# UCSC-VLAA/CLIPA

Measured on AMD Instinct MI355X. Metric: image-text pairs/sec (whole job), full training step, higher is better.
Workload: dtype bf16

## Files before the change

clipa_amd/csrc/attention.hip:

```cpp
#include "common.h"
#include "clipa_hip.h"
#include "attention_common.h"
#include "internal_hooks.h"

namespace {

template <int NKT, int DH, bool CAUSAL>
__global__ __launch_bounds__((64 * attn_waves<NKT, DH>()), HD<DH>::WGS) void attn_fwd_kernel(AttnArgs pin) {
  constexpr int LP = NKT * 32, RB = HD<DH>::RB, KS = HD<DH>::KS, DT = HD<DH>::DT;
  extern __shared__ __attribute__((aligned(16))) char smem[];
  constexpr int HPW = WGHeads<NKT>::HPW, WPH = attn_waves<NKT, DH>() / HPW;
  const int tid = threadIdx.x, lane = tid & 63;
  const int wave_wg = __builtin_amdgcn_readfirstlane(tid >> 6);
  const int slot = wave_wg / WPH, wave = wave_wg % WPH;
  char* sK = smem + slot * (2 * LP * RB);
  char* sV = sK + LP * RB;
  constexpr bool STAGE = fwd_stages<NKT, DH>();
  char* stage = smem + HPW * (2 * LP * RB) + wave_wg * Stg<DH>::BYTES;
  const int l31 = lane & 31, hi = lane >> 5, q16 = (lane >> 4) & 1, i16 = lane & 15;
  const long nheads = (long)pin.B * pin.H;
  const long head_raw = (long)blockIdx.x * HPW + slot;
  const bool live = head_raw < nheads;
  const long head = live ? head_raw : nheads - 1;
  const int b = (int)(head / pin.H), h = (int)(head - (long)b * pin.H);
// ... 67 lines not shown

template <int NKT, int DH, bool CAUSAL>
__global__ __launch_bounds__((64 * attn_waves<NKT, DH>()), HD<DH>::WGS) void attn_bwd_kernel(AttnArgs pin) {
  constexpr int LP = NKT * 32, RB = HD<DH>::RB, KS = HD<DH>::KS, DT = HD<DH>::DT;
  extern __shared__ __attribute__((aligned(16))) char smem[];
  constexpr int HPW = WGHeads<NKT>::HPW, WPH = attn_waves<NKT, DH>() / HPW;
  constexpr bool FENCE = DH == 80 && NKT >= 5;
  const int tid = threadIdx.x, lane = tid & 63;
  const int wave_wg = __builtin_amdgcn_readfirstlane(tid >> 6);
  const int slot = wave_wg / WPH, wave = wave_wg % WPH;
  char* img0 = smem + slot * (2 * LP * RB + 3 * LP * 4);
  char* img1 = img0 + LP * RB;
  float* sM = (float*)(img0 + 2 * LP * RB);
  float* sD = sM + 2 * LP;
  constexpr bool STAGE = bwd_stages<NKT, DH>();
  char* stage = smem + HPW * (2 * LP * RB + 3 * LP * 4) + wave_wg * Stg<DH>::BYTES;
  const int l31 = lane & 31, hi = lane >> 5, q16 = (lane >> 4) & 1, i16 = lane & 15;
  const long nheads = (long)pin.B * pin.H;
  const long head_raw = (long)blockIdx.x * HPW + slot;
  const bool live = head_raw < nheads;
  const long head = live ? head_raw : nheads - 1;
  const int b = (int)(head / pin.H), h = (int)(head - (long)b * pin.H);
  ATTN_LOCATE_SEQUENCE
  const size_t hoff = ((size_t)row0 * p.ld_qkv + (size_t)h * DH) * 2;
  const size_t ooff = ((size_t)row0 * p.ld_o + (size_t)h * DH) * 2;
  const unsigned nrec = (unsigned)((long)(p.L - 1) * p.ld_qkv * 2 + DH * 2);
  const unsigned nrec_o = (unsigned)((long)(p.L - 1) * p.ld_o * 2 + DH * 2);
  const __amdgpu_buffer_rsrc_t rsQ = make_rsrc(p.q + hoff, nrec), rsK = make_rsrc(p.k + hoff, nrec),
                               rsV = make_rsrc(p.v + hoff, nrec), rsDO = make_rsrc(p.d_o + ooff, nrec_o),
                               rsO = make_rsrc(p.o_in + ooff, nrec_o);
  const float c = p.scale * 1.4426950408889634f;
  const float* stats = p.stats + stat0 * 2;

  dma_image<DH>(rsK, img0, LP, p.ld_qkv, wave, lane, WPH);
  dma_image<DH>(rsV, img1, LP, p.ld_qkv, wave, lane, WPH);
  bf16x8 fq[KS], fdo[KS], fo[KS];
  load_frags<KS, DH>(rsQ, p.ld_qkv, 32 * wave + l31, hi, fq);
  load_frags<KS, DH>(rsDO, p.ld_o, 32 * wave + l31, hi, fdo);
  load_frags<KS, DH>(rsO, p.ld_o, 32 * wave + l31, hi, fo);
  asm volatile("s_waitcnt vmcnt(0)" ::: "memory");
  __syncthreads();
  for (int qt = wave; qt < NKT; qt += WPH) {
    const int qg = 32 * qt + l31;
    if (qt != wave) {
      load_frags<KS, DH>(rsQ, p.ld_qkv, qg, hi, fq);
      load_frags<KS, DH>(rsDO, p.ld_o, qg, hi, fdo);
      load_frags<KS, DH>(rsO, p.ld_o, qg, hi, fo);
    }
    float mp = 1e30f;
    if (qg < p.L) {
      const float2 st = *(const float2*)(stats + qg * 2);
      mp = st.x - __builtin_amdgcn_logf(st.y);
    }
    float Dq = 0.f;
#pragma unroll
    for (int ks = 0; ks < KS; ++ks) {
      float a[8], o8[8];
      unpack8(__builtin_bit_cast(u32x4, fdo[ks]), a);
      unpack8(__builtin_bit_cast(u32x4, fo[ks]), o8);
#pragma unroll
      for (int i = 0; i < 8; ++i) Dq += a[i] * o8[i];
    }
    Dq += __shfl_xor(Dq, 32, 64);
    if (hi == 0) { sM[qg] = mp; sD[qg] = Dq; }
    const int lim2 = (CAUSAL ? min(p.L, qg + 1) : p.L) - 4 * hi;
    f32x16 dq[DT];
#pragma unroll
    for (int dt = 0; dt < DT; ++dt)
#pragma unroll
      for (int r = 0; r < 16; ++r) dq[dt][r] = 0.f;
#pragma unroll
    for (int kt = 0; kt < NKT; ++kt) {
      if (CAUSAL && kt > qt) continue;
      f32x16 s, dp;
#pragma unroll
      for (int r = 0; r < 16; ++r) { s[r] = 0.f; dp[r] = 0.f; }
#pragma unroll
      for (int ks = 0; ks < KS; ++ks) {
        s = __builtin_amdgcn_mfma_f32_32x32x16_bf16(frag_direct<DH>(img0, 32 * kt, l31, hi, ks), fq[ks], s, 0, 0, 0);
        dp = __builtin_amdgcn_mfma_f32_32x32x16_bf16(frag_direct<DH>(img1, 32 * kt, l31, hi, ks), fdo[ks], dp, 0, 0, 0);
      }
      if constexpr (FENCE) __builtin_amdgcn_sched_barrier(0);
      const bool full = CAUSAL ? ((32 * kt + 32 <= p.L) && kt < qt) : (kt < NKT - 1);
      float ds[16];
#pragma unroll
      for (int r = 0; r < 16; ++r) {
        float pe = __builtin_amdgcn_exp2f(fmaf(s[r], c, -mp));
        if (!full) pe = (32 * kt + 8 * (r >> 2) + (r & 3) < lim2) ? pe : 0.f;
        ds[r] = pe * (dp[r] - Dq);
      }
      if constexpr (FENCE) __builtin_amdgcn_sched_barrier(0);
#pragma unroll
      for (int s2 = 0; s2 < 2; ++s2) {
        const bf16x8 dsf = pack_frag(ds + 8 * s2);
#pragma unroll
        for (int dt = 0; dt < DT; ++dt)
          dq[dt] = __builtin_amdgcn_mfma_f32_32x32x16_bf16(frag_trans<DH>(img0, 32 * kt + 16 * s2, 32 * dt, hi, q16, i16), dsf, dq[dt], 0, 0, 0);
      }
    }
    if constexpr (STAGE) {
      if (live) store_tile<DH>(stage, p.dq, p.ld_dqkv, row0 + 32 * qt, p.L - 32 * qt, h * DH, lane, dq, p.scale);
    } else if (qg < p.L && live) {
#pragma unroll
      for (int dt = 0; dt < DT; ++dt)
        store_frag_T(p.dq, p.ld_dqkv, row0 + qg, h * DH + 32 * dt, hi, dq[dt], p.scale, DH - 32 * dt);
    }
  }
  bf16x8 fk[KS], fv[KS];
#pragma unroll
  for (int ks = 0; ks < KS; ++ks) {
    fk[ks] = frag_direct<DH>(img0, 32 * min(wave, NKT - 1), l31, hi, ks);
    fv[ks] = frag_direct<DH>(img1, 32 * min(wave, NKT - 1), l31, hi, ks);
  }
  asm volatile("s_waitcnt lgkmcnt(0)" ::: "memory");
  __syncthreads();

  dma_image<DH>(rsQ, img0, LP, p.ld_qkv, wave, lane, WPH);
  dma_image<DH>(rsDO, img1, LP, p.ld_o, wave, lane, WPH);
  asm volatile("s_waitcnt vmcnt(0)" ::: "memory");
  __syncthreads();
  for (int kt = wave; kt < NKT; kt += WPH) {
    const int kg = 32 * kt + l31;
    const int kgc = l31 - 4 * hi;
    if (kt != wave) {
      load_frags<KS, DH>(rsK, p.ld_qkv, kg, hi, fk);
      load_frags<KS, DH>(rsV, p.ld_qkv, kg, hi, fv);
    }
    f32x16 dk[DT], dv[DT];
#pragma unroll
    for (int dt = 0; dt < DT; ++dt)
#pragma unroll
      for (int r = 0; r < 16; ++r) { dk[dt][r] = 0.f; dv[dt][r] = 0.f; }
    for (int qt = (CAUSAL ? kt : 0); qt < NKT; ++qt) {
      f32x16 s, dp;
#pragma unroll
      for (int r = 0; r < 16; ++r) { s[r] = 0.f; dp[r] = 0.f; }
#pragma unroll
      for (int ks = 0; ks < KS; ++ks) {
        s = __builtin_amdgcn_mfma_f32_32x32x16_bf16(frag_direct<DH>(img0, 32 * qt, l31, hi, ks), fk[ks], s, 0, 0, 0);
        dp = __builtin_amdgcn_mfma_f32_32x32x16_bf16(frag_direct<DH>(img1, 32 * qt, l31, hi, ks), fv[ks], dp, 0, 0, 0);
      }
      if constexpr (FENCE) __builtin_amdgcn_sched_barrier(0);
      float pr[16], ds[16];
#pragma unroll
      for (int rq = 0; rq < 4; ++rq) {
        const int q0 = 32 * qt + 8 * rq + 4 * hi;
        const float4 m4 = *(const float4*)(sM + q0);
        const float4 d4 = *(const float4*)(sD + q0);
        const float mm[4] = {m4.x, m4.y, m4.z, m4.w};
        const float dd[4] = {d4.x, d4.y, d4.z, d4.w};
#pragma unroll
        for (int e = 0; e < 4; ++e) {
          const int r = 4 * rq + e;
          float pe = __builtin_amdgcn_exp2f(fmaf(s[r], c, -mm[e]));
          if (CAUSAL && qt == kt) pe = (kgc <= 8 * rq + e) ? pe : 0.f;
          pr[r] = pe;
          ds[r] = pe * (dp[r] - dd[e]);
        }
      }
      if constexpr (FENCE) __builtin_amdgcn_sched_barrier(0);
#pragma unroll
      for (int s2 = 0; s2 < 2; ++s2) {
        const bf16x8 pf = pack_frag(pr + 8 * s2);
        const bf16x8 dsf = pack_frag(ds + 8 * s2);
#pragma unroll
        for (int dt = 0; dt < DT; ++dt) {
          dv[dt] = __builtin_amdgcn_mfma_f32_32x32x16_bf16(frag_trans<DH>(img1, 32 * qt + 16 * s2, 32 * dt, hi, q16, i16), pf, dv[dt], 0, 0, 0);
          dk[dt] = __builtin_amdgcn_mfma_f32_32x32x16_bf16(frag_trans<DH>(img0, 32 * qt + 16 * s2, 32 * dt, hi, q16, i16), dsf, dk[dt], 0, 0, 0);
        }
      }
    }
    if constexpr (STAGE) {
      if (live) {
        store_tile<DH>(stage, p.dk, p.ld_dqkv, row0 + 32 * kt, p.L - 32 * kt, h * DH, lane, dk, p.scale);
        store_tile<DH>(stage, p.dv, p.ld_dqkv, row0 + 32 * kt, p.L - 32 * kt, h * DH, lane, dv, 1.0f);
      }
    } else if (kg < p.L && live) {
#pragma unroll
      for (int dt = 0; dt < DT; ++dt) {
        store_frag_T(p.dk, p.ld_dqkv, row0 + kg, h * DH + 32 * dt, hi, dk[dt], p.scale, DH - 32 * dt);
        store_frag_T(p.dv, p.ld_dqkv, row0 + kg, h * DH + 32 * dt, hi, dv[dt], 1.0f, DH - 32 * dt);
      }
    }
  }
}

constexpr int LONG_CT = 8;
constexpr int LONG_LMAX = 1024;

template <int DH>
__device__ __forceinline__ __amdgpu_buffer_rsrc_t chunk_rsrc(const char* base, long ld, int row0, int L) {
  const long rows = (long)L - row0;
  const long bytes = rows > 0 ? (rows - 1) * ld * 2 + DH * 2 : 0;
  return make_rsrc(base + (size_t)row0 * ld * 2, (unsigned)bytes);
}

template <int DH, bool CAUSAL>
__global__ __launch_bounds__(256, HD<DH>::WGS) void attn_fwd_long_kernel(AttnArgs p) {
  constexpr int CT = LONG_CT, RB = HD<DH>::RB, KS = HD<DH>::KS, DT = HD<DH>::DT;
  extern __shared__ __attribute__((aligned(16))) char smem[];
  const int tid = threadIdx.x, lane = tid & 63;
  const int wave = __builtin_amdgcn_readfirstlane(tid >> 6);
  char* sK = smem;
// ... 320 lines not shown
  if (L <= 0 || L > LONG_LMAX) { clipa_set_error("attention: L=%ld outside (0, %d]", (long)L, LONG_LMAX); return CLIPA_ERR_ARG; }
  if (ld_qkv % 8 != 0 || ld_o % 8 != 0) { clipa_set_error("attention: row strides must be multiples of 8 elements"); return CLIPA_ERR_ARG; }
  if (B * H <= 0 || B * H > 0x7fffffffL) { clipa_set_error("attention: bad B*H"); return CLIPA_ERR_ARG; }
  return 0;
}

}

#define ATTN_DISPATCH_DH(fn, DH, a, st)                                     \
  switch (((a).L + 31) / 32) {                                               \
    case 1: return fn<1, DH>(a, st); case 2: return fn<2, DH>(a, st);        \
    case 3: return fn<3, DH>(a, st); case 4: return fn<4, DH>(a, st);        \
    case 5: return fn<5, DH>(a, st); case 6: return fn<6, DH>(a, st);        \
    case 7: return fn<7, DH>(a, st); case 8: return fn<8, DH>(a, st);        \
    default: return fn<9, DH>(a, st);                                        \
  }
#ifdef CLIPA_ATTN_WIDE
template <int NKT, int DH> int wide_fwd(const AttnArgs& a, hipStream_t st) { return launch_fwd_c<NKT, DH, false>(a, st); }
template <int NKT, int DH> int wide_bwd(const AttnArgs& a, hipStream_t st) { return launch_bwd_c<NKT, DH, false>(a, st); }
template <int DH>
int wide_dh(const AttnArgs& a, int bwd, hipStream_t st) {
  if (a.L > 288) return bwd ? launch_long<DH, false, true>(a, st) : launch_long<DH, false, false>(a, st);
  if (bwd) { ATTN_DISPATCH_DH(wide_bwd, DH, a, st) }
  ATTN_DISPATCH_DH(wide_fwd, DH, a, st)
}
extern "C" int clipa_attn_wide_launch(const void* args, int64_t dh, int bwd, void* stream) {
  const AttnArgs& a = *(const AttnArgs*)args;
  if (dh == 88) return wide_dh<88>(a, bwd, (hipStream_t)stream);
  if (dh == 104) return wide_dh<104>(a, bwd, (hipStream_t)stream);
  return wide_dh<112>(a, bwd, (hipStream_t)stream);
}
#else
extern "C" int clipa_attn_wide_launch(const void* args, int64_t dh, int bwd, void* stream);
#ifdef CLIPA_ATTN_PERSISTENT_EXPERIMENT
extern "C" int clipa_attn_bwd1_try(const void* args, int64_t dh, void* stream, int* rc);
extern "C" int clipa_attn_fwd1_try(const void* args, int64_t dh, void* stream, int* rc);
#endif

#define ATTN_DISPATCH(fn, dh, a, st)                 \
  if ((dh) == 80) { ATTN_DISPATCH_DH(fn, 80, a, st) } \
  ATTN_DISPATCH_DH(fn, 64, a, st)

extern "C" int clipa_attention_fwd(const void* q, const void* k, const void* v, void* out, float* stats,
                                   int64_t B, int64_t H, int64_t L, int64_t dh, int64_t ld_qkv, int64_t ld_o,
                                   float scale, int causal, void* stream) {
  if (B * H == 0) return CLIPA_OK;
  if (int rc = check_args(B, H, L, dh, ld_qkv, ld_o, causal)) return rc;
  AttnArgs a = {};
  a.q = (const char*)q; a.k = (const char*)k; a.v = (const char*)v; a.ld_qkv = ld_qkv;
  a.o = (char*)out; a.ld_o = ld_o; a.B = (int)B; a.H = (int)H; a.L = (int)L; a.scale = scale; a.causal = causal;
  a.stats = stats;
  if (wide_head(dh)) return clipa_attn_wide_launch(&a, dh, 0, stream);
  if (L > 288) return dispatch_long<false>(a, dh, (hipStream_t)stream);
#ifdef CLIPA_ATTN_PERSISTENT_EXPERIMENT
  int rc1 = 0;
  if ((clipa_internal_debug_flags() & 524288) && clipa_attn_fwd1_try(&a, dh, stream, &rc1)) return rc1;
#endif
  ATTN_DISPATCH(launch_fwd, dh, a, (hipStream_t)stream)
}

extern "C" int clipa_attention_bwd(const void* q, const void* k, const void* v, const void* out,
                                   const void* d_out, const float* stats, void* dq, void* dk, void* dv, int64_t B, int64_t H,
                                   int64_t L, int64_t dh, int64_t ld_qkv, int64_t ld_o, int64_t ld_dqkv,
                                   float scale, int causal, void* stream) {
  if (B * H == 0) return CLIPA_OK;
  if (int rc = check_args(B, H, L, dh, ld_qkv, ld_o, causal)) return rc;
  if (ld_dqkv % 8 != 0) { clipa_set_error("attention_bwd: ld_dqkv must be a multiple of 8"); return CLIPA_ERR_ARG; }
  if (!stats) { clipa_set_error("attention_bwd: needs the forward's softmax statistics"); return CLIPA_ERR_ARG; }
  AttnArgs a = {};
  a.q = (const char*)q; a.k = (const char*)k; a.v = (const char*)v; a.ld_qkv = ld_qkv;
  a.o_in = (const char*)out; a.d_o = (const char*)d_out; a.ld_o = ld_o;
  a.dq = (char*)dq; a.dk = (char*)dk; a.dv = (char*)dv; a.ld_dqkv = ld_dqkv;
  a.B = (int)B; a.H = (int)H; a.L = (int)L; a.scale = scale; a.causal = causal;
  a.stats = const_cast<float*>(stats);
  if (wide_head(dh)) return clipa_attn_wide_launch(&a, dh, 1, stream);
  if (L > 288) return dispatch_long<true>(a, dh, (hipStream_t)stream);
#ifdef CLIPA_ATTN_PERSISTENT_EXPERIMENT
  int rc1 = 0;
  if ((clipa_internal_debug_flags() & 262144) && clipa_attn_bwd1_try(&a, dh, stream, &rc1)) return rc1;
#endif
  ATTN_DISPATCH(launch_bwd, dh, a, (hipStream_t)stream)
}
namespace {
int varlen_args(const int* seq_start, const int* seq_len, int64_t nseq, int64_t tiles, int64_t dh) {
  if (!seq_start || !seq_len) { clipa_set_error("attention (varlen): seq_start / seq_len missing"); return CLIPA_ERR_ARG; }
  if (tiles < 1 || tiles > 9) { clipa_set_error("attention (varlen): tiles=%ld outside [1, 9] (sequences of up to 288 tokens)", (long)tiles); return CLIPA_ERR_ARG; }
  if (dh != 64 && dh != 80) { clipa_set_error("attention (varlen): head dim %ld unsupported (64 and 80)", (long)dh); return CLIPA_ERR_ARG; }
  (void)nseq;
  return 0;
}
}

extern "C" int clipa_attention_fwd_varlen(const void* q, const void* k, const void* v, void* out, float* stats,
                                          const int32_t* seq_start, const int32_t* seq_len, const int32_t* seq_ids, int64_t nseq,
                                          int64_t tiles, int64_t H, int64_t dh, int64_t ld_qkv, int64_t ld_o, float scale,
                                          int causal, void* stream) {
  if (nseq * H == 0) return CLIPA_OK;
  if (int rc = check_args(nseq, H, 32 * tiles, dh, ld_qkv, ld_o, causal)) return rc;
  if (int rc = varlen_args(seq_start, seq_len, nseq, tiles, dh)) return rc;
  AttnArgs a = {};
  a.q = (const char*)q; a.k = (const char*)k; a.v = (const char*)v; a.ld_qkv = ld_qkv;
  a.o = (char*)out; a.ld_o = ld_o; a.B = (int)nseq; a.H = (int)H; a.L = (int)(32 * tiles); a.scale = scale; a.causal = causal;
  a.stats = stats;
  a.seq_start = seq_start; a.seq_len = seq_len; a.seq_ids = seq_ids;
  ATTN_DISPATCH(launch_fwd, dh, a, (hipStream_t)stream)
}

extern "C" int clipa_attention_bwd_varlen(const void* q, const void* k, const void* v, const void* out, const void* d_out,
                                          const float* stats, void* dq, void* dk, void* dv, const int32_t* seq_start,
                                          const int32_t* seq_len, const int32_t* seq_ids, int64_t nseq, int64_t tiles, int64_t H,
                                          int64_t dh, int64_t ld_qkv, int64_t ld_o, int64_t ld_dqkv, float scale, int causal,
                                          void* stream) {
  if (nseq * H == 0) return CLIPA_OK;
// ... 15 lines not shown
```

clipa_amd/csrc/attention_common.h:

```cpp
#pragma once
#include "common.h"

namespace {

struct AttnArgs {
  const char* q; const char* k; const char* v; long ld_qkv;
  char* o; const char* o_in; const char* d_o; long ld_o;
  char* dq; char* dk; char* dv; long ld_dqkv;
  float* stats;
  int B, H, L;
  float scale;
  int causal;
  const int* seq_start; const int* seq_len; const int* seq_ids;
  int abl;
};

template <int DH>
struct HD {
  static constexpr int RB = DH == 64 ? 128 : 256;
  static constexpr int NCH = RB / 16;
  static constexpr int KS = (DH + 15) / 16;
  static constexpr int DT = (DH + 31) / 32;
  static constexpr int WGS = DH == 64 ? 2 : 1;
};
template <int NKT>
struct WGHeads {
  static constexpr int HPW = NKT == 1 ? 4 : (NKT == 2 ? 2 : 1);
  static constexpr int WPH = 4 / HPW;
};
template <int NKT, int DH>
__host__ __device__ constexpr int attn_waves() { return (DH == 80 && NKT >= 5) ? 8 : 4; }

template <int DH>
__device__ __forceinline__ int swz_u(int row) {
  if (DH == 64) return (((row >> 1) & 1) << 2) | ((row >> 2) & 1) | (((row >> 3) & 1) << 1);
  return ((row & 3) << 2) | ((row >> 2) & 3);
}

template <int DH>
__device__ __forceinline__ void dma_image(const __amdgpu_buffer_rsrc_t rs, char* img, int LP, long ld,
                                          int wave, int lane, int nwaves = 4) {
  constexpr int NCH = HD<DH>::NCH, RPP = 1024 / HD<DH>::RB;
  for (int pc = wave; pc < LP / RPP; pc += nwaves) {
    const int row = pc * RPP + lane / NCH;
    const int chunk = (lane & (NCH - 1)) ^ swz_u<DH>(row);
    const unsigned oob = (chunk * 8 >= DH) ? 0x80000000u : 0u;
    __builtin_amdgcn_raw_ptr_buffer_load_lds(rs, LDS_PTR(img + pc * 1024), 16,
                                             (unsigned)(row * ld * 2 + chunk * 16) | oob, 0, 0, 0);
  }
}

template <int DH>
__device__ __forceinline__ bf16x8 frag_direct(const char* img, int rowbase, int l31, int hi, int ks) {
  return *(const bf16x8*)(img + (rowbase + l31) * HD<DH>::RB + (((2 * ks + hi) ^ swz_u<DH>(l31)) << 4));
}

template <int DH>
__device__ __forceinline__ bf16x8 frag_trans(const char* img, int rowbase16, int colbase, int hi, int q16, int i16) {
  constexpr int RB = HD<DH>::RB;
  const int col = colbase + 16 * q16 + 4 * (i16 & 3);
  const int r0 = rowbase16 + 4 * hi + (i16 >> 2);
  const int r1 = r0 + 8;
  const bf16x4 a = __builtin_amdgcn_ds_read_tr16_b64_v4i16(
      (__attribute__((address_space(3))) bf16x4*)(img + r0 * RB + (((col >> 3) ^ swz_u<DH>(r0)) << 4) + (col & 7) * 2));
  const bf16x4 b = __builtin_amdgcn_ds_read_tr16_b64_v4i16(
      (__attribute__((address_space(3))) bf16x4*)(img + r1 * RB + (((col >> 3) ^ swz_u<DH>(r1)) << 4) + (col & 7) * 2));
  bf16x8 f;
  f[0] = a[0]; f[1] = a[1]; f[2] = a[2]; f[3] = a[3];
  f[4] = b[0]; f[5] = b[1]; f[6] = b[2]; f[7] = b[3];
  return f;
}

__device__ __forceinline__ bf16x8 pack_frag(const float* v) {
  u32x4 w;
#pragma unroll
  for (int i = 0; i < 4; ++i) w[i] = pack2bf(v[2 * i], v[2 * i + 1]);
  return __builtin_bit_cast(bf16x8, w);
}

__device__ __forceinline__ void store_frag_T(char* base, long ld, long row, int col0, int hi, const f32x16& a, float mul,
                                             int ncols = 32) {
#pragma unroll
  for (int qd = 0; qd < 4; ++qd) {
    if (8 * qd >= ncols) continue;
// ... 136 lines not shown
```

clipa_amd/csrc/misc.hip:

```cpp
#include "common.h"
#include "stream.h"
#include "clipa_hip.h"

namespace {

template <int DT>
__global__ void patchify_kernel(const void* __restrict__ img, unsigned short* __restrict__ out,
                                int B, int S, int P, int g, int Kp, int nhwc, int normalize,
                                float m0, float m1, float m2, float is0, float is1, float is2) {
  const long total = (long)B * g * g * (Kp / 8);
  const int K = 3 * P * P;
  const bool fast8 = nhwc && (3 * P) % 8 == 0 && (3 * S) % 8 == 0 && ((size_t)img & 7) == 0;
  for (long idx = (long)blockIdx.x * blockDim.x + threadIdx.x; idx < total; idx += (long)gridDim.x * blockDim.x) {
    const int kc = (int)(idx % (Kp / 8));
    const long patch = idx / (Kp / 8);
    const int px = (int)(patch % g);
    const int py = (int)((patch / g) % g);
    const long b = patch / ((long)g * g);
    float f[8];
    if (DT == 0 && fast8) {
      const int k0 = kc * 8;
      if (k0 < K) {
        const int ph = k0 / (3 * P), off = k0 - ph * 3 * P;
        const size_t src = (((size_t)b * S + (py * P + ph)) * S + px * P) * 3 + off;
// ... 103 lines not shown
template <bool TBF16>
__global__ void embed_tokens_kernel(const long* __restrict__ ids, const void* __restrict__ table,
                                    const float* __restrict__ pos, unsigned short* __restrict__ out,
                                    long B, int T, int D, int vocab, int* __restrict__ oob) {
  const int dc = D / 8;
  const long total = B * T * dc;
  for (long idx = (long)blockIdx.x * blockDim.x + threadIdx.x; idx < total; idx += (long)gridDim.x * blockDim.x) {
    const int c = (int)(idx % dc);
    const long row = idx / dc;
    const int t = (int)(row % T);
    long id = ids[row];
    if (id < 0 || id >= vocab) {
      if (c == 0 && oob) atomicAdd(oob, 1);
      id = 0;
    }
    float v[8], pe[8];
    if (TBF16) {
      unpack8(*(const u32x4*)((const unsigned short*)table + (size_t)id * D + c * 8), v);
    } else {
      *(float4*)v = *(const float4*)((const float*)table + (size_t)id * D + c * 8);
      *(float4*)(v + 4) = *(const float4*)((const float*)table + (size_t)id * D + c * 8 + 4);
#pragma unroll
      for (int i = 0; i < 8; ++i) v[i] = bf2f(f2bf(v[i]));
    }
    *(float4*)pe = *(const float4*)(pos + (size_t)t * D + c * 8);
    *(float4*)(pe + 4) = *(const float4*)(pos + (size_t)t * D + c * 8 + 4);
#pragma unroll
    for (int i = 0; i < 8; ++i) v[i] += bf2f(f2bf(pe[i]));
    *(u32x4*)(out + (size_t)row * D + c * 8) = pack8(v);
  }
}

constexpr double EMB_FIX = 17592186044416.0;
__global__ void embed_tokens_bwd_kernel(const long* __restrict__ ids, const unsigned short* __restrict__ dx,
                                        unsigned long long* __restrict__ acc, unsigned char* __restrict__ bad_row, long B, int T,
                                        int D, int vocab, int* __restrict__ oob) {
  const int dc = D / 8;
  const long total = B * T * dc;
  for (long idx = (long)blockIdx.x * blockDim.x + threadIdx.x; idx < total; idx += (long)gridDim.x * blockDim.x) {
    const int c = (int)(idx % dc);
    const long row = idx / dc;
    const long id = ids[row];
    if (id < 0 || id >= vocab) {
      if (c == 0 && oob) atomicAdd(oob, 1);
      continue;
    }
    const u32x4 raw = *(const u32x4*)(dx + (size_t)row * D + c * 8);
    if (((raw[0] | raw[1] | raw[2] | raw[3]) & 0x7fff7fffu) == 0) continue;
    float v[8];
    unpack8(raw, v);
#pragma unroll
    for (int i = 0; i < 8; ++i) {
      if (v[i] == 0.f) continue;
      if (!(fabsf(v[i]) <= 3.0e38f)) { bad_row[id] = 1; continue; }
      const float vs = fminf(fmaxf(v[i], -131072.0f), 131072.0f);
      atomicAdd(acc + (size_t)id * D + c * 8 + i, (unsigned long long)__double2ll_rn((double)vs * EMB_FIX));
    }
  }
}
__global__ void embed_fix_to_f32_kernel(const long long* __restrict__ acc, const unsigned char* __restrict__ bad_row,
                                        float* __restrict__ out, long n, int D) {
  for (long i = (long)blockIdx.x * blockDim.x + threadIdx.x; i < n; i += (long)gridDim.x * blockDim.x)
    out[i] = bad_row[i / D] ? __int_as_float(0x7fc00000) : (float)((double)acc[i] * (1.0 / EMB_FIX));
}

__global__ void argmax_tokens_kernel(const long* __restrict__ ids, int* __restrict__ out, long B, int T) {
  const long b = (long)blockIdx.x * blockDim.x + threadIdx.x;
  if (b >= B) return;
  long best = ids[b * T];
  int bi = 0;
  for (int t = 1; t < T; ++t) {
    const long v = ids[b * T + t];
    if (v > best) { best = v; bi = t; }
  }
  out[b] = bi;
}

__global__ void pool_fwd_kernel(const unsigned short* __restrict__ x, const int* __restrict__ idx,
                                float* __restrict__ out, long B, int L, int D, int mode) {
  const int dc = D / 8;
  const long total = B * dc;
  for (long i = (long)blockIdx.x * blockDim.x + threadIdx.x; i < total; i += (long)gridDim.x * blockDim.x) {
    const int c = (int)(i % dc);
    const long b = i / dc;
    float acc[8] = {0, 0, 0, 0, 0, 0, 0, 0};
    int l0, l1;
    if (mode == CLIPA_POOL_FIRST) { l0 = 0; l1 = 1; }
    else if (mode == CLIPA_POOL_LAST) { l0 = L - 1; l1 = L; }
    else if (mode == CLIPA_POOL_INDEX) { l0 = idx[b]; l1 = l0 + 1; }
    else if (mode == CLIPA_POOL_MEAN_ALL) { l0 = 0; l1 = L; }
    else { l0 = 1; l1 = L; }
    for (int l = l0; l < l1; ++l) {
      float v[8];
      unpack8(*(const u32x4*)(x + ((size_t)b * L + l) * D + c * 8), v);
#pragma unroll
      for (int k = 0; k < 8; ++k) acc[k] += v[k];
// ... 228 lines not shown
extern "C" int clipa_assemble_tokens_bwd(const void* dtokens, void* dpatch, float* dcls, float* dpos,
                                         int64_t B, int64_t L, int64_t D, void* workspace, int64_t workspace_bytes,
                                         void* stream) {
  if (D % 8 != 0) { clipa_set_error("assemble_tokens_bwd: D%%8 != 0"); return CLIPA_ERR_ARG; }
  if (B <= 0) return CLIPA_OK;
  if (!workspace || workspace_bytes < clipa_assemble_tokens_bwd_workspace(B, L, D)) { clipa_set_error("assemble_tokens_bwd: workspace too small"); return CLIPA_ERR_ARG; }
  hipStream_t st = (hipStream_t)stream;
  int nchunk, bchunk;
  assemble_bwd_chunks(B, L, D, &nchunk, &bchunk);
  const long threads = L * (D / 8);
  hipLaunchKernelGGL(assemble_tokens_bwd_kernel, dim3((unsigned)((threads + 255) / 256), (unsigned)nchunk), dim3(256), 0, st,
                     (const unsigned short*)dtokens, (unsigned short*)dpatch, (float*)workspace, (long)B, (int)L, (int)D, bchunk);
  if (int rc = clipa_check_launch("assemble_tokens_bwd")) return rc;
  if (!dcls && !dpos) return CLIPA_OK;
  const long n = dpos ? L * D : D;
  hipLaunchKernelGGL(assemble_tokens_bwd_reduce_kernel, dim3((unsigned)((n + 255) / 256)), dim3(256), 0, st, (const float*)workspace,
                     dcls, dpos, (int)L, (int)D, nchunk);
  return clipa_check_launch("assemble_tokens_bwd_reduce");
}

extern "C" int clipa_embed_tokens(const int64_t* ids, const void* table, int table_bf16, const float* pos,
                                  void* out, int64_t B, int64_t T, int64_t D, int64_t vocab, int32_t* oob_count,
                                  void* stream) {
  if (D % 8 != 0) { clipa_set_error("embed_tokens: D%%8 != 0"); return CLIPA_ERR_ARG; }
  if (B <= 0) return CLIPA_OK;
  const unsigned grid = grid_for(B * T * (D / 8));
  if (table_bf16) hipLaunchKernelGGL(embed_tokens_kernel<true>, dim3(grid), dim3(256), 0, (hipStream_t)stream, (const long*)ids, table, pos, (unsigned short*)out, (long)B, (int)T, (int)D, (int)vocab, oob_count);
  else hipLaunchKernelGGL(embed_tokens_kernel<false>, dim3(grid), dim3(256), 0, (hipStream_t)stream, (const long*)ids, table, pos, (unsigned short*)out, (long)B, (int)T, (int)D, (int)vocab, oob_count);
  return clipa_check_launch("embed_tokens");
}

extern "C" int64_t clipa_embed_tokens_bwd_workspace(int64_t B, int64_t T, int64_t D, int64_t vocab, int need_table,
                                                   int need_pos) {
  int64_t w = need_table ? vocab * D * (int64_t)sizeof(long long) + (vocab + 7) / 8 * 8 : 0;
  const int64_t pw = need_pos ? clipa_assemble_tokens_bwd_workspace(B, T, D) : 0;
  return w > pw ? w : pw;
}

extern "C" int clipa_embed_tokens_bwd(const int64_t* ids, const void* dx, float* dtable, float* dpos,
                                      int64_t B, int64_t T, int64_t D, int64_t vocab, int32_t* oob_count, void* workspace,
                                      int64_t workspace_bytes, void* stream) {
  if (D % 8 != 0) { clipa_set_error("embed_tokens_bwd: D%%8 != 0"); return CLIPA_ERR_ARG; }
  if (B <= 0) return CLIPA_OK;
  if (!workspace || workspace_bytes < clipa_embed_tokens_bwd_workspace(B, T, D, vocab, dtable != nullptr, dpos != nullptr)) {
    clipa_set_error("embed_tokens_bwd: workspace too small");
    return CLIPA_ERR_ARG;
  }
  hipStream_t st = (hipStream_t)stream;
  if (dtable) {
    unsigned char* bad_row = (unsigned char*)workspace + vocab * D * sizeof(long long);
    (void)hipMemsetAsync(workspace, 0, vocab * D * sizeof(long long) + (vocab + 7) / 8 * 8, st);
    hipLaunchKernelGGL(embed_tokens_bwd_kernel, dim3(grid_for(B * T * (D / 8))), dim3(256), 0, st, (const long*)ids, (const unsigned short*)dx, (unsigned long long*)workspace, bad_row, (long)B, (int)T, (int)D, (int)vocab, oob_count);
    if (int rc = clipa_check_launch("embed_tokens_bwd")) return rc;
    hipLaunchKernelGGL(embed_fix_to_f32_kernel, dim3(grid_for(vocab * D)), dim3(256), 0, st, (const long long*)workspace, bad_row, dtable, (long)(vocab * D), (int)D);
    if (int rc = clipa_check_launch("embed_tokens_bwd_convert")) return rc;
  }
  if (dpos) return clipa_assemble_tokens_bwd(dx, nullptr, nullptr, dpos, B, T, D, workspace, workspace_bytes, stream);
  return CLIPA_OK;
}

extern "C" int clipa_argmax_tokens(const int64_t* ids, int32_t* out, int64_t B, int64_t T, void* stream) {
  if (B <= 0) return CLIPA_OK;
  hipLaunchKernelGGL(argmax_tokens_kernel, dim3((unsigned)((B + 255) / 256)), dim3(256), 0, (hipStream_t)stream, (const long*)ids, out, (long)B, (int)T);
  return clipa_check_launch("argmax_tokens");
}

extern "C" int clipa_pool_fwd(const void* x, const int32_t* idx, float* out, int64_t B, int64_t L, int64_t D,
                              int mode, void* stream) {
  if (D % 8 != 0 || (mode == CLIPA_POOL_INDEX && !idx)) { clipa_set_error("pool_fwd: bad args"); return CLIPA_ERR_ARG; }
  if (B <= 0) return CLIPA_OK;
  hipLaunchKernelGGL(pool_fwd_kernel, dim3(grid_for(B * (D / 8))), dim3(256), 0, (hipStream_t)stream, (const unsigned short*)x, idx, out, (long)B, (int)L, (int)D, mode);
  return clipa_check_launch("pool_fwd");
}
extern "C" int clipa_pool_bwd(const float* dout, const int32_t* idx, void* dx, int64_t B, int64_t L, int64_t D,
                              int mode, void* stream) {
  if (D % 8 != 0 || (mode == CLIPA_POOL_INDEX && !idx)) { clipa_set_error("pool_bwd: bad args"); return CLIPA_ERR_ARG; }
  if (B <= 0) return CLIPA_OK;
  hipLaunchKernelGGL(pool_bwd_kernel, dim3(grid_for(B * L * (D / 8))), dim3(256), 0, (hipStream_t)stream, dout, idx, (unsigned short*)dx, (long)B, (int)L, (int)D, mode);
  return clipa_check_launch("pool_bwd");
}

namespace {
__global__ void gather_rows_kernel(const unsigned short* __restrict__ x, const int64_t* __restrict__ rows,
                                   unsigned short* __restrict__ out, long n_out, long n_src, int D) {
  const int dc = D / 8;
  const long total = n_out * dc;
  for (long idx = (long)blockIdx.x * blockDim.x + threadIdx.x; idx < total; idx += (long)gridDim.x * blockDim.x) {
    const long r = idx / dc;
// ... 252 lines not shown
```

Before: 2468.

## Prefetch next tile fragments and use direct-to-LDS DMA in attention backward

Measured after the change: 2473, median of 6. No clear change (+0.2%).

```diff
diff --git a/clipa_amd/csrc/attention.hip b/clipa_amd/csrc/attention.hip
--- a/clipa_amd/csrc/attention.hip
+++ b/clipa_amd/csrc/attention.hip
@@ -123,8 +123,9 @@
   const float c = p.scale * 1.4426950408889634f;
   const float* stats = p.stats + stat0 * 2;
 
-  dma_image<DH>(rsK, img0, LP, p.ld_qkv, wave, lane, WPH);
-  dma_image<DH>(rsV, img1, LP, p.ld_qkv, wave, lane, WPH);
+  constexpr bool HIDDEN = attn_bwd_hidden_dma<NKT, DH, CAUSAL>();
+  head_image<DH, LP, WPH, HIDDEN>(p.k + hoff, nrec, img0, p.ld_qkv, wave, lane);
+  head_image<DH, LP, WPH, HIDDEN>(p.v + hoff, nrec, img1, p.ld_qkv, wave, lane);
   bf16x8 fq[KS], fdo[KS], fo[KS];
   load_frags<KS, DH>(rsQ, p.ld_qkv, 32 * wave + l31, hi, fq);
   load_frags<KS, DH>(rsDO, p.ld_o, 32 * wave + l31, hi, fdo);
@@ -133,7 +134,7 @@
   __syncthreads();
   for (int qt = wave; qt < NKT; qt += WPH) {
     const int qg = 32 * qt + l31;
-    if (qt != wave) {
+    if (!HIDDEN && qt != wave) {
       load_frags<KS, DH>(rsQ, p.ld_qkv, qg, hi, fq);
       load_frags<KS, DH>(rsDO, p.ld_o, qg, hi, fdo);
       load_frags<KS, DH>(rsO, p.ld_o, qg, hi, fo);
@@ -188,6 +189,11 @@
         for (int dt = 0; dt < DT; ++dt)
           dq[dt] = __builtin_amdgcn_mfma_f32_32x32x16_bf16(frag_trans<DH>(img0, 32 * kt + 16 * s2, 32 * dt, hi, q16, i16), dsf, dq[dt], 0, 0, 0);
       }
+    }
+    if (HIDDEN && qt + WPH < NKT) {
+      load_frags<KS, DH>(rsQ, p.ld_qkv, qg + 32 * WPH, hi, fq);
+      load_frags<KS, DH>(rsDO, p.ld_o, qg + 32 * WPH, hi, fdo);
+      load_frags<KS, DH>(rsO, p.ld_o, qg + 32 * WPH, hi, fo);
     }
     if constexpr (STAGE) {
       if (live) store_tile<DH>(stage, p.dq, p.ld_dqkv, row0 + 32 * qt, p.L - 32 * qt, h * DH, lane, dq, p.scale);
@@ -206,14 +212,14 @@
   asm volatile("s_waitcnt lgkmcnt(0)" ::: "memory");
   __syncthreads();
 
-  dma_image<DH>(rsQ, img0, LP, p.ld_qkv, wave, lane, WPH);
-  dma_image<DH>(rsDO, img1, LP, p.ld_o, wave, lane, WPH);
+  head_image<DH, LP, WPH, HIDDEN>(p.q + hoff, nrec, img0, p.ld_qkv, wave, lane);
+  head_image<DH, LP, WPH, HIDDEN>(p.d_o + ooff, nrec_o, img1, p.ld_o, wave, lane);
   asm volatile("s_waitcnt vmcnt(0)" ::: "memory");
   __syncthreads();
   for (int kt = wave; kt < NKT; kt += WPH) {
     const int kg = 32 * kt + l31;
     const int kgc = l31 - 4 * hi;
-    if (kt != wave) {
+    if (!HIDDEN && kt != wave) {
       load_frags<KS, DH>(rsK, p.ld_qkv, kg, hi, fk);
       load_frags<KS, DH>(rsV, p.ld_qkv, kg, hi, fv);
     }
@@ -260,6 +266,10 @@
           dk[dt] = __builtin_amdgcn_mfma_f32_32x32x16_bf16(frag_trans<DH>(img0, 32 * qt + 16 * s2, 32 * dt, hi, q16, i16), dsf, dk[dt], 0, 0, 0);
         }
       }
+    }
+    if (HIDDEN && kt + WPH < NKT) {
+      load_frags<KS, DH>(rsK, p.ld_qkv, kg + 32 * WPH, hi, fk);
+      load_frags<KS, DH>(rsV, p.ld_qkv, kg + 32 * WPH, hi, fv);
     }
     if constexpr (STAGE) {
       if (live) {
@@ -646,10 +656,6 @@
 }
 #else
 extern "C" int clipa_attn_wide_launch(const void* args, int64_t dh, int bwd, void* stream);
-#ifdef CLIPA_ATTN_PERSISTENT_EXPERIMENT
-extern "C" int clipa_attn_bwd1_try(const void* args, int64_t dh, void* stream, int* rc);
-extern "C" int clipa_attn_fwd1_try(const void* args, int64_t dh, void* stream, int* rc);
-#endif
 
 #define ATTN_DISPATCH(fn, dh, a, st)                 \
   if ((dh) == 80) { ATTN_DISPATCH_DH(fn, 80, a, st) } \
@@ -666,10 +672,6 @@
   a.stats = stats;
   if (wide_head(dh)) return clipa_attn_wide_launch(&a, dh, 0, stream);
   if (L > 288) return dispatch_long<false>(a, dh, (hipStream_t)stream);
-#ifdef CLIPA_ATTN_PERSISTENT_EXPERIMENT
-  int rc1 = 0;
-  if ((clipa_internal_debug_flags() & 524288) && clipa_attn_fwd1_try(&a, dh, stream, &rc1)) return rc1;
-#endif
   ATTN_DISPATCH(launch_fwd, dh, a, (hipStream_t)stream)
 }
 
@@ -689,10 +691,6 @@
   a.stats = const_cast<float*>(stats);
   if (wide_head(dh)) return clipa_attn_wide_launch(&a, dh, 1, stream);
   if (L > 288) return dispatch_long<true>(a, dh, (hipStream_t)stream);
-#ifdef CLIPA_ATTN_PERSISTENT_EXPERIMENT
-  int rc1 = 0;
-  if ((clipa_internal_debug_flags() & 262144) && clipa_attn_bwd1_try(&a, dh, stream, &rc1)) return rc1;
-#endif
   ATTN_DISPATCH(launch_bwd, dh, a, (hipStream_t)stream)
 }
 namespace {
diff --git a/clipa_amd/csrc/attention_common.h b/clipa_amd/csrc/attention_common.h
--- a/clipa_amd/csrc/attention_common.h
+++ b/clipa_amd/csrc/attention_common.h
@@ -1,5 +1,6 @@
 #pragma once
 #include "common.h"
+#include "gemm_common.h"
 
 namespace {
 
@@ -12,7 +13,6 @@
   float scale;
   int causal;
   const int* seq_start; const int* seq_len; const int* seq_ids;
-  int abl;
 };
 
 template <int DH>
@@ -50,6 +50,34 @@
   }
 }
 
+template <int NKT, int DH, bool CAUSAL>
+__host__ __device__ constexpr bool attn_bwd_hidden_dma() { return DH == 64 && NKT >= 3 && !(NKT == 8 && !CAUSAL); }
+
+template <int DH, int LP, int NWAVES>
+__device__ __forceinline__ void dma_image_hidden(const u32x4 srd, char* img, long ld, int wave, int lane) {
+  constexpr int NCH = HD<DH>::NCH, RPP = 1024 / HD<DH>::RB, PIECES = LP / RPP;
+  static_assert(PIECES % NWAVES == 0, "every wave issues the same number of pieces");
+#pragma unroll
+  for (int j = 0; j < PIECES / NWAVES; ++j) {
+    const int pc = wave + j * NWAVES;
+    const int row = pc * RPP + lane / NCH;
+    const int chunk = (lane & (NCH - 1)) ^ swz_u<DH>(row);
+    const unsigned oob = (chunk * 8 >= DH) ? 0x80000000u : 0u;
+    clipa_gemm::dma16(srd, (unsigned)(size_t)LDS_PTR(img + pc * 1024), (unsigned)(row * ld * 2 + chunk * 16) | oob, 0u);
+  }
+}
+template <int DH, int LP, int NWAVES, bool HIDDEN>
+__device__ __forceinline__ void head_image(const char* base, unsigned nrec, char* img, long ld, int wave, int lane) {
+  if constexpr (HIDDEN) {
+    u32x4 srd = clipa_gemm::make_srd(base, nrec);
+#pragma unroll
+    for (int i = 0; i < 4; ++i) srd[i] = __builtin_amdgcn_readfirstlane(srd[i]);
+    dma_image_hidden<DH, LP, NWAVES>(srd, img, ld, wave, lane);
+  } else {
+    dma_image<DH>(make_rsrc(base, nrec), img, LP, ld, wave, lane, NWAVES);
+  }
+}
+
 template <int DH>
 __device__ __forceinline__ bf16x8 frag_direct(const char* img, int rowbase, int l31, int hi, int ks) {
   return *(const bf16x8*)(img + (rowbase + l31) * HD<DH>::RB + (((2 * ks + hi) ^ swz_u<DH>(l31)) << 4));
```

## Replace atomic fixed-point embedding backward with sort-by-token segmented reduction

Applied to the files above, without the earlier changes.

New measurement: 2476 before, 2482 after, median of 6. About the same (+0.2%).

```diff
diff --git a/clipa_amd/csrc/misc.hip b/clipa_amd/csrc/misc.hip
--- a/clipa_amd/csrc/misc.hip
+++ b/clipa_amd/csrc/misc.hip
@@ -159,36 +159,223 @@
 }
 
 constexpr double EMB_FIX = 17592186044416.0;
-__global__ void embed_tokens_bwd_kernel(const long* __restrict__ ids, const unsigned short* __restrict__ dx,
-                                        unsigned long long* __restrict__ acc, unsigned char* __restrict__ bad_row, long B, int T,
-                                        int D, int vocab, int* __restrict__ oob) {
+constexpr int EMB_SEG = 32;
+
+struct EmbBwdWs {
+  int* count;
+  unsigned char* bad;
+  int* rowoff;
+  int* itemoff;
+  int* slotoff;
+  int* item_id;
+  int* rank;
+  int* sorted;
+  long long* partial;
+  int64_t zero_bytes, bytes;
+};
+inline EmbBwdWs emb_bwd_carve(void* ws, int64_t nrows, int64_t D, int64_t vocab) {
+  EmbBwdWs w;
+  int64_t off = 0;
+  auto take = [&](int64_t bytes) { void* p = (void*)((uintptr_t)ws + (uintptr_t)off); off += (bytes + 15) / 16 * 16; return p; };
+  w.count = (int*)take(vocab * 4);
+  w.bad = (unsigned char*)take(vocab);
+  w.zero_bytes = off;
+  w.rowoff = (int*)take((vocab + 1) * 4);
+  w.itemoff = (int*)take((vocab + 1) * 4);
+  w.slotoff = (int*)take((vocab + 1) * 4);
+  w.item_id = (int*)take((vocab + nrows / EMB_SEG) * 4);
+  w.rank = (int*)take(nrows * 4);
+  w.sorted = (int*)take(nrows * 4);
+  w.partial = (long long*)take((2 * nrows / EMB_SEG + 1) * D * (int64_t)sizeof(long long));
+  w.bytes = off;
+  return w;
+}
+
+__global__ void embed_bwd_count_kernel(const long* __restrict__ ids, const unsigned short* __restrict__ dx,
+                                       int* __restrict__ count, int* __restrict__ rank, long nrows, int D, int vocab,
+                                       int* __restrict__ oob) {
+  const int lane = threadIdx.x & 63;
+  const long row = (long)blockIdx.x * blockDim.x + threadIdx.x;
+  const long wbase = row - lane;
   const int dc = D / 8;
-  const long total = B * T * dc;
+  const int nr = (int)(nrows - wbase < 64 ? nrows - wbase : 64);
+  bool live = false;
+#pragma unroll 4
+  for (int k = 0; k < nr; ++k) {
+    unsigned any = 0;
+    for (int c = lane; c < dc; c += 64) {
+      const u32x4 raw = *(const u32x4*)(dx + (size_t)(wbase + k) * D + c * 8);
+      any |= (raw[0] | raw[1] | raw[2] | raw[3]) & 0x7fff7fffu;
+    }
+    const bool nz = __ballot(any != 0) != 0ull;
+    if (lane == k) live = nz;
+  }
+  int id = -1;
+  if (row < nrows) {
+    const long id64 = ids[row];
+    if (id64 < 0 || id64 >= vocab) { if (oob) atomicAdd(oob, 1); }
+    else if (live) id = (int)id64;
+  }
+  int leader = lane, within = 0, gsize = 1;
+  bool todo = id >= 0;
+  for (unsigned long long pending = __ballot(todo); pending; pending = __ballot(todo)) {
+    const int first = __ffsll((long long)pending) - 1;
+    const bool mine = todo && id == __shfl(id, first);
+    const unsigned long long grp = __ballot(mine);
+    if (mine) {
+      leader = first;
+      within = __popcll(grp & ((1ull << lane) - 1ull));
+      gsize = __popcll(grp);
+      todo = false;
+    }
+  }
+  int base = 0;
+  if (id >= 0 && lane == leader) base = atomicAdd(count + id, gsize);
+  base = __shfl(base, leader);
+  if (row < nrows) rank[row] = id >= 0 ? base + within : -1;
+}
+
+__device__ __forceinline__ void emb_block_scan3(int (&v)[3], int (*s)[1024]) {
+  const int t = threadIdx.x;
+#pragma unroll
+  for (int k = 0; k < 3; ++k) s[k][t] = v[k];
+  __syncthreads();
+  for (int d = 1; d < 1024; d <<= 1) {
+    int u[3];
+#pragma unroll
+    for (int k = 0; k < 3; ++k) u[k] = t >= d ? s[k][t - d] : 0;
+    __syncthreads();
+#pragma unroll
+    for (int k = 0; k < 3; ++k) s[k][t] += u[k];
+    __syncthreads();
+  }
+#pragma unroll
+  for (int k = 0; k < 3; ++k) v[k] = s[k][t];
+}
+__device__ __forceinline__ void emb_id_sizes(int n, int (&v)[3]) {
+  const int items = n > EMB_SEG ? (n + EMB_SEG - 1) / EMB_SEG : 1;
+  v[0] = n; v[1] = items; v[2] = items > 1 ? items : 0;
+}
+
+__global__ __launch_bounds__(1024) void embed_bwd_scan_kernel(const int* __restrict__ count, int* __restrict__ rowoff,
+                                                              int* __restrict__ itemoff, int* __restrict__ slotoff,
+                                                              int* __restrict__ item_id, int vocab) {
+  __shared__ int s[3][1024];
+  const int t = threadIdx.x, first = blockIdx.x * 1024, id = first + t;
+  int front[3] = {0, 0, 0};
+  for (int i = t; i < first; i += 1024) {
+    int v[3];
+    emb_id_sizes(count[i], v);
+#pragma unroll
+    for (int k = 0; k < 3; ++k) front[k] += v[k];
+  }
+  emb_block_scan3(front, s);
+  int base[3];
+#pragma unroll
+  for (int k = 0; k < 3; ++k) base[k] = s[k][1023];
+  __syncthreads();
+  int own[3] = {0, 0, 0}, incl[3];
+  if (id < vocab) emb_id_sizes(count[id], own);
+#pragma unroll
+  for (int k = 0; k < 3; ++k) incl[k] = own[k];
+  emb_block_scan3(incl, s);
+  if (id >= vocab) return;
+  const int r = base[0] + incl[0] - own[0], it = base[1] + incl[1] - own[1], sl = base[2] + incl[2] - own[2];
+  rowoff[id] = r;
+  itemoff[id] = it;
+  slotoff[id] = sl;
+  for (int j = 0; j < own[1]; ++j) item_id[it + j] = id;
+  if (id == vocab - 1) { rowoff[vocab] = r + own[0]; itemoff[vocab] = it + own[1]; slotoff[vocab] = sl + own[2]; }
+}
+
+__global__ void embed_bwd_place_kernel(const long* __restrict__ ids, const int* __restrict__ rank,
+                                       const int* __restrict__ rowoff, int* __restrict__ sorted, long nrows) {
+  const long row = (long)blockIdx.x * blockDim.x + threadIdx.x;
+  if (row >= nrows) return;
+  const int r = rank[row];
+  if (r >= 0) sorted[rowoff[ids[row]] + r] = (int)row;
+}
+
+__device__ __forceinline__ void emb_fix_add(const u32x4 raw, long long (&acc)[8], bool& nonfinite) {
+  if (((raw[0] | raw[1] | raw[2] | raw[3]) & 0x7fff7fffu) == 0) return;
+  float v[8];
+  unpack8(raw, v);
+#pragma unroll
+  for (int i = 0; i < 8; ++i) {
+    if (v[i] == 0.f) continue;
+    if (!(fabsf(v[i]) <= 3.0e38f)) { nonfinite = true; continue; }
+    const float vs = fminf(fmaxf(v[i], -131072.0f), 131072.0f);
+    acc[i] = (long long)((unsigned long long)acc[i] + (unsigned long long)__double2ll_rn((double)vs * EMB_FIX));
+  }
+}
+__device__ __forceinline__ void emb_fix_store(const long long (&acc)[8], float* __restrict__ out) {
+  float f[8];
+#pragma unroll
+  for (int i = 0; i < 8; ++i) f[i] = (float)((double)acc[i] * (1.0 / EMB_FIX));
+  *(float4*)out = make_float4(f[0], f[1], f[2], f[3]);
+  *(float4*)(out + 4) = make_float4(f[4], f[5], f[6], f[7]);
+}
+
+__global__ void embed_bwd_sum_kernel(const unsigned short* __restrict__ dx, const int* __restrict__ rowoff,
+                                     const int* __restrict__ itemoff, const int* __restrict__ slotoff,
+                                     const int* __restrict__ item_id, const int* __restrict__ sorted,
+                                     unsigned char* __restrict__ bad, long long* __restrict__ partial,
+                                     float* __restrict__ dtable, int D, int vocab) {
+  const int item = blockIdx.x;
+  if (item >= itemoff[vocab]) return;
+  const int id = item_id[item];
+  const int j = item - itemoff[id], nitems = itemoff[id + 1] - itemoff[id];
+  const int r0 = rowoff[id] + j * EMB_SEG;
+  const int r1 = r0 + EMB_SEG < rowoff[id + 1] ? r0 + EMB_SEG : rowoff[id + 1];
+  const int dc = D / 8;
+  for (int c = threadIdx.x; c < dc; c += blockDim.x) {
+    long long acc[8] = {0, 0, 0, 0, 0, 0, 0, 0};
+    bool nonfinite = false;
+    for (int r = r0; r < r1; r += 4) {
+      u32x4 raw[4];
+#pragma unroll
+      for (int u = 0; u < 4; ++u) {
+        raw[u] = u32x4{0u, 0u, 0u, 0u};
+        if (r + u < r1) raw[u] = *(const u32x4*)(dx + (size_t)sorted[r + u] * D + c * 8);
+      }
+#pragma unroll
+      for (int u = 0; u < 4; ++u) emb_fix_add(raw[u], acc, nonfinite);
+    }
+    if (nonfinite) bad[id] = 1;
+    if (nitems == 1) {
+      emb_fix_store(acc, dtable + (size_t)id * D + c * 8);
+    } else {
+      long long* p = partial + (size_t)(slotoff[id] + j) * D + c * 8;
+#pragma unroll
+      for (int i = 0; i < 8; ++i) p[i] = acc[i];
+    }
+  }
+}
+
+__global__ void embed_bwd_merge_kernel(const int* __restrict__ itemoff, const int* __restrict__ slotoff,
+                                       const unsigned char* __restrict__ bad, const long long* __restrict__ partial,
+                                       float* __restrict__ dtable, int D, int vocab) {
+  const int dc = D / 8;
+  const long total = (long)vocab * dc;
   for (long idx = (long)blockIdx.x * blockDim.x + threadIdx.x; idx < total; idx += (long)gridDim.x * blockDim.x) {
     const int c = (int)(idx % dc);
-    const long row = idx / dc;
-    const long id = ids[row];
-    if (id < 0 || id >= vocab) {
-      if (c == 0 && oob) atomicAdd(oob, 1);
-      continue;
-    }
-    const u32x4 raw = *(const u32x4*)(dx + (size_t)row * D + c * 8);
-    if (((raw[0] | raw[1] | raw[2] | raw[3]) & 0x7fff7fffu) == 0) continue;
-    float v[8];
-    unpack8(raw, v);
-#pragma unroll
-    for (int i = 0; i < 8; ++i) {
-      if (v[i] == 0.f) continue;
-      if (!(fabsf(v[i]) <= 3.0e38f)) { bad_row[id] = 1; continue; }
-      const float vs = fminf(fmaxf(v[i], -131072.0f), 131072.0f);
-      atomicAdd(acc + (size_t)id * D + c * 8 + i, (unsigned long long)__double2ll_rn((double)vs * EMB_FIX));
-    }
-  }
-}
-__global__ void embed_fix_to_f32_kernel(const long long* __restrict__ acc, const unsigned char* __restrict__ bad_row,
-                                        float* __restrict__ out, long n, int D) {
-  for (long i = (long)blockIdx.x * blockDim.x + threadIdx.x; i < n; i += (long)gridDim.x * blockDim.x)
-    out[i] = bad_row[i / D] ? __int_as_float(0x7fc00000) : (float)((double)acc[i] * (1.0 / EMB_FIX));
+    const int id = (int)(idx / dc);
+    const int nitems = itemoff[id + 1] - itemoff[id];
+    float* out = dtable + (size_t)id * D + c * 8;
+    if (bad[id]) {
+      const float nan = __int_as_float(0x7fc00000);
+      *(float4*)out = make_float4(nan, nan, nan, nan);
+      *(float4*)(out + 4) = make_float4(nan, nan, nan, nan);
+    } else if (nitems > 1) {
+      long long acc[8] = {0, 0, 0, 0, 0, 0, 0, 0};
+      const long long* p = partial + (size_t)slotoff[id] * D + c * 8;
+      for (int j = 0; j < nitems; ++j, p += D) {
+#pragma unroll
+        for (int i = 0; i < 8; ++i) acc[i] = (long long)((unsigned long long)acc[i] + (unsigned long long)p[i]);
+      }
+      emb_fix_store(acc, out);
+    }
+  }
 }
 
 __global__ void argmax_tokens_kernel(const long* __restrict__ ids, int* __restrict__ out, long B, int T) {
@@ -483,7 +670,7 @@
 
 extern "C" int64_t clipa_embed_tokens_bwd_workspace(int64_t B, int64_t T, int64_t D, int64_t vocab, int need_table,
                                                    int need_pos) {
-  int64_t w = need_table ? vocab * D * (int64_t)sizeof(long long) + (vocab + 7) / 8 * 8 : 0;
+  int64_t w = need_table ? emb_bwd_carve(nullptr, B * T, D, vocab).bytes : 0;
   const int64_t pw = need_pos ? clipa_assemble_tokens_bwd_workspace(B, T, D) : 0;
   return w > pw ? w : pw;
 }
@@ -499,12 +686,21 @@
   }
   hipStream_t st = (hipStream_t)stream;
   if (dtable) {
-    unsigned char* bad_row = (unsigned char*)workspace + vocab * D * sizeof(long long);
-    (void)hipMemsetAsync(workspace, 0, vocab * D * sizeof(long long) + (vocab + 7) / 8 * 8, st);
-    hipLaunchKernelGGL(embed_tokens_bwd_kernel, dim3(grid_for(B * T * (D / 8))), dim3(256), 0, st, (const long*)ids, (const unsigned short*)dx, (unsigned long long*)workspace, bad_row, (long)B, (int)T, (int)D, (int)vocab, oob_count);
+    const int64_t nrows = B * T;
+    if (vocab <= 0 || nrows + vocab >= 0x7fffffffLL) { clipa_set_error("embed_tokens_bwd: B*T + vocab does not fit 32-bit row indices"); return CLIPA_ERR_ARG; }
+    const EmbBwdWs w = emb_bwd_carve(workspace, nrows, D, vocab);
+    (void)hipMemsetAsync(w.count, 0, w.zero_bytes, st);
+    hipLaunchKernelGGL(embed_bwd_count_kernel, dim3(grid_for(nrows)), dim3(256), 0, st, (const long*)ids, (const unsigned short*)dx, w.count, w.rank, (long)nrows, (int)D, (int)vocab, oob_count);
+    if (int rc = clipa_check_launch("embed_tokens_bwd_count")) return rc;
+    hipLaunchKernelGGL(embed_bwd_scan_kernel, dim3((unsigned)((vocab + 1023) / 1024)), dim3(1024), 0, st, (const int*)w.count, w.rowoff, w.itemoff, w.slotoff, w.item_id, (int)vocab);
+    if (int rc = clipa_check_launch("embed_tokens_bwd_scan")) return rc;
+    hipLaunchKernelGGL(embed_bwd_place_kernel, dim3(grid_for(nrows)), dim3(256), 0, st, (const long*)ids, (const int*)w.rank, (const int*)w.rowoff, w.sorted, (long)nrows);
+    if (int rc = clipa_check_launch("embed_tokens_bwd_place")) return rc;
+    const int dc = (int)(D / 8), threads = dc >= 256 ? 256 : (dc + 63) / 64 * 64;
+    hipLaunchKernelGGL(embed_bwd_sum_kernel, dim3((unsigned)(vocab + nrows / EMB_SEG)), dim3(threads), 0, st, (const unsigned short*)dx, (const int*)w.rowoff, (const int*)w.itemoff, (const int*)w.slotoff, (const int*)w.item_id, (const int*)w.sorted, w.bad, w.partial, dtable, (int)D, (int)vocab);
     if (int rc = clipa_check_launch("embed_tokens_bwd")) return rc;
-    hipLaunchKernelGGL(embed_fix_to_f32_kernel, dim3(grid_for(vocab * D)), dim3(256), 0, st, (const long long*)workspace, bad_row, dtable, (long)(vocab * D), (int)D);
-    if (int rc = clipa_check_launch("embed_tokens_bwd_convert")) return rc;
+    hipLaunchKernelGGL(embed_bwd_merge_kernel, dim3(grid_for(vocab * dc, 256, 8192)), dim3(256), 0, st, (const int*)w.itemoff, (const int*)w.slotoff, (const unsigned char*)w.bad, (const long long*)w.partial, dtable, (int)D, (int)vocab);
+    if (int rc = clipa_check_launch("embed_tokens_bwd_merge")) return rc;
   }
   if (dpos) return clipa_assemble_tokens_bwd(dx, nullptr, nullptr, dpos, B, T, D, workspace, workspace_bytes, stream);
   return CLIPA_OK;
```
